# zhanxw/rvtests

Hardware: AMD Instinct MI355X
Metric: gene-sets/sec (SKAT+SKAT-O+CMC+Zeggini, analytic p-values) (higher is better)
Workload: dtype f64

## Files before the change

### rvtests_amd/csrc/k2_hardcall.hip

```cpp
#include "suffstat_hc.hip.h"

namespace rvt {

void k2_launch_hc(int MT, dim3 grid, hipStream_t st, const GeneDesc* d_desc, NullTile nt, long long N, long long ld,
                  int d) {
  switch (MT) {
    case 1: hipLaunchKernelGGL((gene_suffstat_hc<1, 2, 4, false>), grid, dim3(64), 0, st, d_desc, nt, N, ld, d); break;
    case 2: hipLaunchKernelGGL((gene_suffstat_hc<2, 2, 3, false>), grid, dim3(64), 0, st, d_desc, nt, N, ld, d); break;
    case 3: hipLaunchKernelGGL((gene_suffstat_hc<3, 2, 2, false>), grid, dim3(64), 0, st, d_desc, nt, N, ld, d); break;
    case 4: hipLaunchKernelGGL((gene_suffstat_hc<4, 2, 2, false>), grid, dim3(64), 0, st, d_desc, nt, N, ld, d); break;
    case 5: hipLaunchKernelGGL((gene_suffstat_hc<5, 1, 1, false>), grid, dim3(64), 0, st, d_desc, nt, N, ld, d); break;
    case 6: hipLaunchKernelGGL((gene_suffstat_hc<6, 1, 1, false>), grid, dim3(64), 0, st, d_desc, nt, N, ld, d); break;
    default: break;
  }
}

void k2_launch_classify(dim3 grid, hipStream_t st, const double* G, long long N, long long ld, int M, int* flag) {
  hipLaunchKernelGGL(block_classify_kernel<0>, grid, dim3(256), 0, st, G, N, ld, M, flag);
}

}
```

### rvtests_amd/csrc/suffstat_hc.hip.h

```cpp
#pragma once
#include <type_traits>
#include "suffstat_kernels.hip.h"

namespace rvt {

typedef int i4_t __attribute__((ext_vector_type(4)));
typedef unsigned int u4_t __attribute__((ext_vector_type(4)));

constexpr int kHcMaxMT = 6;
constexpr int kHcMaxD = 13;
constexpr int kHcStepUnit = 12;
constexpr int kHcMaxSteps = 1020;
constexpr int kHcColstatRows = 6;

constexpr int hc_pq_tiles(int MT) { return MT * MT + MT * (MT + 1) / 2; }
constexpr int hc_pq_words(int MT) { return hc_pq_tiles(MT) * 128; }
constexpr int hc_lds_words(int MT) { return hc_pq_words(MT) + 64 * MT + 4; }

struct NullTile {
  const double* base;
  int cols;
};

__device__ __forceinline__ unsigned row16_sum(unsigned h) {
  h += (unsigned)__builtin_amdgcn_update_dpp(0, (int)h, 0xB1, 0xF, 0xF, true);
  h += (unsigned)__builtin_amdgcn_update_dpp(0, (int)h, 0x4E, 0xF, 0xF, true);
  h += (unsigned)__builtin_amdgcn_update_dpp(0, (int)h, 0x141, 0xF, 0xF, true);
  h += (unsigned)__builtin_amdgcn_update_dpp(0, (int)h, 0x140, 0xF, 0xF, true);
  return h;
}

template <int MT>
struct HcStep {
  u4_t glo[MT], ghi[MT];
  u4_t xlo, xhi;
};

template <int MT, bool NT>
__device__ __forceinline__ void hc_issue(HcStep<MT>& f, const __amdgpu_buffer_rsrc_t& rg, const unsigned (&voff)[MT],
                                         const __amdgpu_buffer_rsrc_t& rx, unsigned xoff, int imm) {
#pragma unroll
  for (int c = 0; c < MT; ++c) {
    f.glo[c] = __builtin_bit_cast(u4_t, __builtin_amdgcn_raw_buffer_load_b128(rg, voff[c] + imm, 0, NT ? 2 : 0));
    f.ghi[c] = __builtin_bit_cast(u4_t, __builtin_amdgcn_raw_buffer_load_b128(rg, voff[c] + imm + 16, 0, NT ? 2 : 0));
  }
  f.xlo = __builtin_bit_cast(u4_t, __builtin_amdgcn_raw_buffer_load_b128(rx, xoff + imm, 0, 0));
  f.xhi = __builtin_bit_cast(u4_t, __builtin_amdgcn_raw_buffer_load_b128(rx, xoff + imm + 16, 0, 0));
}

__device__ __forceinline__ double hc_dbl(unsigned lo, unsigned hi) {
  return __builtin_bit_cast(double, ((unsigned long long)hi << 32) | lo);
}

struct HcBurden {
  double a_cmc, a_zeg;
  unsigned zz, cnt;
};

template <bool MASKED>
__device__ __forceinline__ void hc_row(const u4_t& glo, const u4_t& ghi, const double (&xv)[4], d4_t& accT,
                                       unsigned& pk, unsigned& mk, unsigned& cs, unsigned fx, unsigned& h, bool valid) {
  const double g0 = hc_dbl(glo[0], glo[1]), g1 = hc_dbl(glo[2], glo[3]), g2 = hc_dbl(ghi[0], ghi[1]),
               g3 = hc_dbl(ghi[2], ghi[3]);
  accT = __builtin_amdgcn_mfma_f64_16x16x4f64(g0, xv[0], accT, 0, 0, 0);
  accT = __builtin_amdgcn_mfma_f64_16x16x4f64(g1, xv[1], accT, 0, 0, 0);
  accT = __builtin_amdgcn_mfma_f64_16x16x4f64(g2, xv[2], accT, 0, 0, 0);
  accT = __builtin_amdgcn_mfma_f64_16x16x4f64(g3, xv[3], accT, 0, 0, 0);
  const unsigned w01 = __builtin_amdgcn_perm(glo[3], glo[1], 0x0c0c0703u);
  const unsigned w23 = __builtin_amdgcn_perm(ghi[3], ghi[1], 0x07030c0cu);
  unsigned p = ((w01 | w23) >> 5) & 0x03030303u;
  constexpr unsigned kAdd = 0x00100000u, kBits = 0xBFEFFFFFu;
  const unsigned i0 = ((glo[1] + kAdd) & kBits) | glo[0], i1 = ((glo[3] + kAdd) & kBits) | glo[2],
                 i2 = ((ghi[1] + kAdd) & kBits) | ghi[0], i3 = ((ghi[3] + kAdd) & kBits) | ghi[2];
  auto one = [](unsigned x) { return x < 1u ? x : 1u; };
  unsigned m = one(i0) | (one(i1) << 8) | (one(i2) << 16) | (one(i3) << 24);
  if (MASKED) {
    p = valid ? p : 0u;
    m = valid ? m : 0u;
  }
  const unsigned m3 = m * 3u;
  p &= ~m3;
  pk = p;
  mk = m;
  cs = __builtin_amdgcn_sad_u8(p, 0u, cs);
  const unsigned t = (p ^ fx) & ~m3;
  h += (t | (t >> 1)) & 0x01010101u;
}
__device__ __forceinline__ unsigned hc_code3(unsigned p) { return p & (p >> 1) & 0x01010101u; }

__device__ __forceinline__ void hc_note_masked(const u4_t& glo, const u4_t& ghi, unsigned mk, unsigned* oa) {
  auto note = [&](unsigned lo, unsigned hi) {
    __hip_atomic_fetch_or(oa + 0, lo, __ATOMIC_RELAXED, __HIP_MEMORY_SCOPE_WORKGROUP);
    __hip_atomic_fetch_or(oa + 1, hi, __ATOMIC_RELAXED, __HIP_MEMORY_SCOPE_WORKGROUP);
    __hip_atomic_fetch_and(oa + 2, lo, __ATOMIC_RELAXED, __HIP_MEMORY_SCOPE_WORKGROUP);
    __hip_atomic_fetch_and(oa + 3, hi, __ATOMIC_RELAXED, __HIP_MEMORY_SCOPE_WORKGROUP);
  };
  if (mk & 0x000000ffu) note(glo[0], glo[1]);
  if (mk & 0x0000ff00u) note(glo[2], glo[3]);
  if (mk & 0x00ff0000u) note(ghi[0], ghi[1]);
  if (mk & 0xff000000u) note(ghi[2], ghi[3]);
}

template <bool MASKED>
__device__ __forceinline__ void hc_finish(unsigned h, const double (&xv)[4], HcBurden& bu, unsigned vmask) {
  h = row16_sum(h);
  if (MASKED) h &= vmask;
#pragma unroll
  for (int l = 0; l < 4; ++l) {
    const unsigned cz = (h >> (8 * l)) & 0xffu;
    const unsigned cc = cz ? 1u : 0u;
    bu.zz = cz * cz + bu.zz;
    bu.cnt += cc;
    bu.a_zeg = fma((double)cz, xv[l], bu.a_zeg);
    bu.a_cmc = fma((double)cc, xv[l], bu.a_cmc);
  }
}

struct HcMaskCtx {
  unsigned* oa;
  unsigned* flag;
};

template <int MT, bool MASKED>
__device__ __forceinline__ void hc_step(const HcStep<MT>& f, const int T, d4_t (&accT)[MT], unsigned (&pk)[MT][4],
                                        unsigned (&cs)[MT], const unsigned (&fx)[MT], HcBurden& bu, bool valid,
                                        unsigned vmask, unsigned& anym, const HcMaskCtx& mc) {
  double xv[4] = {hc_dbl(f.xlo[0], f.xlo[1]), hc_dbl(f.xlo[2], f.xlo[3]), hc_dbl(f.xhi[0], f.xhi[1]),
                  hc_dbl(f.xhi[2], f.xhi[3])};
  if (MASKED) {
#pragma unroll
    for (int l = 0; l < 4; ++l) xv[l] = valid ? xv[l] : 0.0;
  }
  unsigned h = 0;
#pragma unroll
  for (int c = 0; c < MT; ++c) {
    unsigned p, m;
    hc_row<MASKED>(f.glo[c], f.ghi[c], xv, accT[c], p, m, cs[c], fx[c], h, valid);
    if (m) hc_note_masked(f.glo[c], f.ghi[c], m, mc.oa + 64 * c);
    if (hc_code3(p)) __hip_atomic_fetch_or(mc.flag, 2u, __ATOMIC_RELAXED, __HIP_MEMORY_SCOPE_WORKGROUP);
    pk[c][T] = p | (m << 2);
    anym |= m;
  }
  hc_finish<MASKED>(h, xv, bu, vmask);
}

template <int MT>
__device__ __forceinline__ void hc_gram(const unsigned (&pk)[MT][4], i4_t (&accS)[MT * (MT + 1) / 2]) {
  i4_t op[MT];
#pragma unroll
  for (int c = 0; c < MT; ++c) op[c] = i4_t{(int)pk[c][0], (int)pk[c][1], (int)pk[c][2], (int)pk[c][3]};
  int t = 0;
#pragma unroll
  for (int r = 0; r < MT; ++r)
#pragma unroll
    for (int c = r; c < MT; ++c, ++t) accS[t] = __builtin_amdgcn_mfma_i32_16x16x64_i8(op[r], op[c], accS[t], 0, 0, 0);
}

template <int MT>
__device__ __forceinline__ void hc_gram_masked(const unsigned (&pk)[MT][4], unsigned* lds, int lane) {
  auto mask_op = [&](int c) {
    return i4_t{(int)((pk[c][0] >> 2) & 0x01010101u), (int)((pk[c][1] >> 2) & 0x01010101u),
                (int)((pk[c][2] >> 2) & 0x01010101u), (int)((pk[c][3] >> 2) & 0x01010101u)};
  };
  auto add = [&](int tile, const i4_t& z) {
    const unsigned w0 = (unsigned)z[0] | ((unsigned)z[1] << 16), w1 = (unsigned)z[2] | ((unsigned)z[3] << 16);
    __hip_atomic_fetch_add(lds + (tile * 2 + 0) * 64 + lane, w0, __ATOMIC_RELAXED, __HIP_MEMORY_SCOPE_WORKGROUP);
    __hip_atomic_fetch_add(lds + (tile * 2 + 1) * 64 + lane, w1, __ATOMIC_RELAXED, __HIP_MEMORY_SCOPE_WORKGROUP);
  };
#pragma unroll
  for (int c = 0; c < MT; ++c) {
    const i4_t mc = mask_op(c);
#pragma unroll
    for (int r = 0; r < MT; ++r) {
      const i4_t a = i4_t{(int)pk[r][0], (int)pk[r][1], (int)pk[r][2], (int)pk[r][3]};
      add(r * MT + c, __builtin_amdgcn_mfma_i32_16x16x64_i8(a, mc, i4_t{0, 0, 0, 0}, 0, 0, 0));
      if (r <= c) {
        const i4_t mr = (r == c) ? mc : mask_op(r);
        add(MT * MT + r * MT - r * (r - 1) / 2 + (c - r), __builtin_amdgcn_mfma_i32_16x16x64_i8(mr, mc, i4_t{0, 0, 0, 0}, 0, 0, 0));
      }
    }
    __builtin_amdgcn_sched_barrier(0);
  }
  __hip_atomic_fetch_or(lds + hc_pq_words(MT) + 64 * MT, 1u, __ATOMIC_RELAXED, __HIP_MEMORY_SCOPE_WORKGROUP);
}

template <int MT>
__device__ __forceinline__ void hc_group_end(const unsigned (&pk)[MT][4], i4_t (&accS)[MT * (MT + 1) / 2], unsigned& anym,
                                             unsigned* lds, int lane) {
  hc_gram<MT>(pk, accS);
  if (__builtin_amdgcn_ballot_w64(anym != 0u) != 0ull) hc_gram_masked<MT>(pk, lds, lane);
  anym = 0u;
}

template <int MT, int DEPTH, bool NT>
__device__ __forceinline__ void suffstat_hc_body(const GeneDesc& gd, const NullTile& nt, long long N, long long ld,
                                                 int d, unsigned* lds) {
  const int lane = threadIdx.x & 63;
  const int v = lane & 15, q = lane >> 4;
  const int wpart = blockIdx.x;
  if (wpart >= gd.n_wparts) return;
  constexpr int kPQ = hc_pq_words(MT);
#pragma unroll 4
  for (int w = lane; w < kPQ; w += 64) lds[w] = 0u;
#pragma unroll
  for (int c = 0; c < MT; ++c) lds[kPQ + 64 * c + lane] = (lane & 2) ? 0xffffffffu : 0u;
  if (lane < 4) lds[kPQ + 64 * MT + lane] = 0u;
  const HcMaskCtx mc{lds + kPQ + 4 * v, lds + kPQ + 64 * MT};
  unsigned anym = 0u;
  const long long nsteps = ld >> 4;
  const long long s_begin = (long long)wpart * gd.steps_per_wpart;
  long long s_end = s_begin + gd.steps_per_wpart;
  if (s_end > nsteps) s_end = nsteps;
  if (s_begin >= s_end) return;
  const int M = gd.M;
  auto uniform = [](const void* p) {
    const unsigned long long a = (unsigned long long)p;
    const unsigned lo = __builtin_amdgcn_readfirstlane((unsigned)a);
    const unsigned hi = __builtin_amdgcn_readfirstlane((unsigned)(a >> 32));
    return (void*)(((unsigned long long)hi << 32) | lo);
  };
  const unsigned gbytes = (unsigned)((unsigned long long)M * (unsigned long long)ld * 8ull);
  const __amdgpu_buffer_rsrc_t rg = __builtin_amdgcn_make_buffer_rsrc(uniform(gd.G), 0, gbytes, 0x00020000);
  const unsigned xbytes = (unsigned)((unsigned long long)nt.cols * (unsigned long long)ld * 8ull);
  const __amdgpu_buffer_rsrc_t rx = __builtin_amdgcn_make_buffer_rsrc(uniform(nt.base), 0, xbytes, 0x00020000);
  const unsigned lane_off = (unsigned)(q * 32);
  const unsigned col_bytes = (unsigned)((unsigned long long)ld * 8ull);
  unsigned vbase[MT];
#pragma unroll
  for (int c = 0; c < MT; ++c) {
    const int col = c * 16 + v;
    vbase[c] = (col < M) ? (unsigned)col * col_bytes + lane_off : 0x80000000u;
  }
  const int xcol = (v <= d) ? v : d + 1;
  const unsigned xbase = (unsigned)xcol * col_bytes + lane_off;
  unsigned fx[MT];
#pragma unroll
  for (int c = 0; c < MT; ++c) fx[c] = ((gd.pflip[c] >> v) & 1) ? 0x02020202u : 0u;

  d4_t accT[MT];
  i4_t accS[MT * (MT + 1) / 2];
  unsigned cs[MT], pk[MT][4];
#pragma unroll
  for (int c = 0; c < MT; ++c) {
    accT[c] = d4_t{0.0, 0.0, 0.0, 0.0};
    cs[c] = 0;
  }
#pragma unroll
  for (int t = 0; t < MT * (MT + 1) / 2; ++t) accS[t] = i4_t{0, 0, 0, 0};
  HcBurden bu{0.0, 0.0, 0u, 0u};

  long long s = s_begin;
  const long long full = N >> 4;
  const long long s_fast_end = (s_end < full) ? s_end : full;
  constexpr int U = (DEPTH == 3) ? 12 : 4;
  const long long n_fast = (s_fast_end > s_begin) ? (s_fast_end - s_begin) / U : 0;
  if constexpr (DEPTH == 1) {
   if (n_fast > 0) {
    unsigned voff[MT];
#pragma unroll
    for (int c = 0; c < MT; ++c) voff[c] = vbase[c] + (unsigned)(s_begin * 128);
    unsigned xoff = xbase + (unsigned)(s_begin * 128);
    u4_t glo[MT], ghi[MT], xlo[2], xhi[2];
#pragma unroll
    for (int c = 0; c < MT; ++c) {
      glo[c] = __builtin_bit_cast(u4_t, __builtin_amdgcn_raw_buffer_load_b128(rg, voff[c], 0, NT ? 2 : 0));
      ghi[c] = __builtin_bit_cast(u4_t, __builtin_amdgcn_raw_buffer_load_b128(rg, voff[c] + 16, 0, NT ? 2 : 0));
    }
    xlo[0] = __builtin_bit_cast(u4_t, __builtin_amdgcn_raw_buffer_load_b128(rx, xoff, 0, 0));
    xhi[0] = __builtin_bit_cast(u4_t, __builtin_amdgcn_raw_buffer_load_b128(rx, xoff + 16, 0, 0));
    for (long long it = 0; it < n_fast; ++it) {
#pragma unroll
      for (int u = 0; u < 4; ++u) {
        xlo[(u + 1) & 1] = __builtin_bit_cast(u4_t, __builtin_amdgcn_raw_buffer_load_b128(rx, xoff + (u + 1) * 128, 0, 0));
        xhi[(u + 1) & 1] = __builtin_bit_cast(u4_t, __builtin_amdgcn_raw_buffer_load_b128(rx, xoff + (u + 1) * 128 + 16, 0, 0));
        __builtin_amdgcn_sched_barrier(0);
        const double xv[4] = {hc_dbl(xlo[u & 1][0], xlo[u & 1][1]), hc_dbl(xlo[u & 1][2], xlo[u & 1][3]),
                              hc_dbl(xhi[u & 1][0], xhi[u & 1][1]), hc_dbl(xhi[u & 1][2], xhi[u & 1][3])};
        unsigned h = 0;
#pragma unroll
        for (int c = 0; c < MT; ++c) {
          unsigned p, m;
          hc_row<false>(glo[c], ghi[c], xv, accT[c], p, m, cs[c], fx[c], h, true);
          if (m) hc_note_masked(glo[c], ghi[c], m, mc.oa + 64 * c);
          if (hc_code3(p)) __hip_atomic_fetch_or(mc.flag, 2u, __ATOMIC_RELAXED, __HIP_MEMORY_SCOPE_WORKGROUP);
          pk[c][u] = p | (m << 2);
          anym |= m;
          glo[c] = __builtin_bit_cast(u4_t, __builtin_amdgcn_raw_buffer_load_b128(rg, voff[c] + (u + 1) * 128, 0, NT ? 2 : 0));
          ghi[c] = __builtin_bit_cast(u4_t, __builtin_amdgcn_raw_buffer_load_b128(rg, voff[c] + (u + 1) * 128 + 16, 0, NT ? 2 : 0));
          __builtin_amdgcn_sched_barrier(0);
        }
        hc_finish<false>(h, xv, bu, 0xffffffffu);
        if (u == 3) hc_group_end<MT>(pk, accS, anym, lds, lane);
        __builtin_amdgcn_sched_barrier(0);
      }
#pragma unroll
      for (int c = 0; c < MT; ++c) voff[c] += 4 * 128;
      xoff += 4 * 128;
    }
    s += n_fast * U;
   }
  } else if (n_fast > 0) {
    unsigned voff[MT];
#pragma unroll
    for (int c = 0; c < MT; ++c) voff[c] = vbase[c] + (unsigned)(s_begin * 128);
    unsigned xoff = xbase + (unsigned)(s_begin * 128);
    HcStep<MT> f[DEPTH];
#pragma unroll
    for (int u = 0; u < DEPTH - 1; ++u) hc_issue<MT, NT>(f[u], rg, voff, rx, xoff, u * 128);
    for (long long it = 0; it < n_fast; ++it) {
#pragma unroll
      for (int u = 0; u < U; ++u) {
        hc_issue<MT, NT>(f[(u + DEPTH - 1) % DEPTH], rg, voff, rx, xoff, (u + DEPTH - 1) * 128);
        __builtin_amdgcn_sched_barrier(0);
        hc_step<MT, false>(f[u % DEPTH], u & 3, accT, pk, cs, fx, bu, true, 0xffffffffu, anym, mc);
        if ((u & 3) == 3) hc_group_end<MT>(pk, accS, anym, lds, lane);
        __builtin_amdgcn_sched_barrier(0);
      }
#pragma unroll
      for (int c = 0; c < MT; ++c) voff[c] += U * 128;
      xoff += U * 128;
    }
    s += n_fast * U;
  }
  while (s < s_end) {
#pragma unroll
    for (int c = 0; c < MT; ++c) pk[c][0] = pk[c][1] = pk[c][2] = pk[c][3] = 0u;
    auto one = [&](const int T, long long su) {
      const bool valid = su < s_end;
      const long long sc = valid ? su : s_end - 1;
      unsigned voff[MT];
#pragma unroll
      for (int c = 0; c < MT; ++c) voff[c] = vbase[c] + (unsigned)(sc * 128);
      HcStep<MT> f;
      hc_issue<MT, false>(f, rg, voff, rx, xbase + (unsigned)(sc * 128), 0);
      unsigned vmask = 0u;
      const long long smp = sc * 16 + q * 4;
#pragma unroll
      for (int l = 0; l < 4; ++l) vmask |= (valid && smp + l < N) ? (0xffu << (8 * l)) : 0u;
      hc_step<MT, true>(f, T, accT, pk, cs, fx, bu, valid, vmask, anym, mc);
    };
    one(0, s);
    one(1, s + 1);
    one(2, s + 2);
    one(3, s + 3);
    hc_group_end<MT>(pk, accS, anym, lds, lane);
    s += 4;
  }

  double* out = gd.parts + (long long)wpart * gd.Mp * gd.Cp;
  const int Cp = gd.Cp;
  {
    int t = 0;
#pragma unroll
    for (int r = 0; r < MT; ++r)
#pragma unroll
      for (int c = r; c < MT; ++c, ++t) {
        const int col = c * 16 + v;
        if (col < M) {
#pragma unroll
          for (int i = 0; i < 4; ++i) out[(long long)(r * 16 + q * 4 + i) * Cp + col] = (double)accS[t][i];
        }
      }
  }
#pragma unroll
  for (int r = 0; r < MT; ++r) {
#pragma unroll
    for (int i = 0; i < 4; ++i) {
      const int row = r * 16 + q + 4 * i;
      if (M + v < Cp) out[(long long)row * Cp + M + v] = accT[r][i];
      if (M + 16 + v < Cp) out[(long long)row * Cp + M + 16 + v] = 0.0;
    }
  }
  long long cnt_w = ((s_end * 16 < N) ? s_end * 16 : N) - s_begin * 16;
  if (cnt_w < 0) cnt_w = 0;
  double* cst = gd.colstat + (long long)wpart * kHcColstatRows * gd.Mp;
  const unsigned wflag = lds[kPQ + 64 * MT];
  {
    int t = 0;
#pragma unroll
    for (int c = 0; c < MT; ++c) {
      unsigned sc = cs[c];
      sc += __shfl_xor(sc, 16, 64);
      sc += __shfl_xor(sc, 32, 64);
      const i4_t dg = accS[t];
      const int sel = (lane & 3) == 0 ? dg[0] : ((lane & 3) == 1 ? dg[1] : ((lane & 3) == 2 ? dg[2] : dg[3]));
      const int diag = __shfl(sel, v + 16 * (v >> 2), 64);
      const int tq = MT * MT + t;
      const unsigned qw = lds[(tq * 2 + ((v >> 1) & 1)) * 64 + v + 16 * (v >> 2)];
      const long long nm = (long long)((qw >> (16 * (v & 1))) & 0xffffu);
      t += MT - c;
      const long long sm = (long long)sc, hh = (long long)diag - 16 * nm, n2 = (hh - sm) / 2, n1 = 2 * sm - hh,
                      n0 = cnt_w - n1 - n2 - nm;
      const double mn = n0 > 0 ? 0.0 : (n1 > 0 ? 1.0 : (n2 > 0 ? 2.0 : INFINITY));
      const double mx = n2 > 0 ? 2.0 : (n1 > 0 ? 1.0 : (n0 > 0 ? 0.0 : -INFINITY));
      if (lane < 16) {
        const int j = c * 16 + lane;
        cst[j] = (double)sm;
        cst[gd.Mp + j] = mn;
        cst[2 * gd.Mp + j] = mx;
        cst[3 * gd.Mp + j] = (double)nm;
        const unsigned* w = lds + kPQ + 64 * c + 4 * lane;
        unsigned long long* bits = reinterpret_cast<unsigned long long*>(cst);
        bits[4 * gd.Mp + j] = ((unsigned long long)w[1] << 32) | w[0];
        bits[5 * gd.Mp + j] = ((unsigned long long)w[3] << 32) | w[2];
      }
    }
  }
  if (gd.wflags && lane == 0) gd.wflags[wpart] = wflag;
  if ((wflag & 1u) && gd.pq) {
    unsigned* dst = gd.pq + (long long)wpart * kPQ;
#pragma unroll 4
    for (int w = lane; w < kPQ; w += 64) dst[w] = lds[w];
  }
  if (gd.bparts) {
    double ac = bu.a_cmc, az = bu.a_zeg;
    ac += __shfl_xor(ac, 16, 64);
    az += __shfl_xor(az, 16, 64);
    ac += __shfl_xor(ac, 32, 64);
    az += __shfl_xor(az, 32, 64);
    unsigned zz = bu.zz, cn = bu.cnt;
    zz += __shfl_xor(zz, 16, 64);
    cn += __shfl_xor(cn, 16, 64);
    zz += __shfl_xor(zz, 32, 64);
    cn += __shfl_xor(cn, 32, 64);
    const int rl = 3 + d;
    double* bp = gd.bparts + (long long)wpart * 2 * rl;
    if (lane <= d) {
      const int k = (lane == d) ? 0 : 3 + lane;
      bp[k] = ac;
      bp[rl + k] = az;
    }
    if (lane == 0) {
      bp[1] = (double)cn;
      bp[2] = (double)cn;
      bp[rl + 1] = (double)zz;
      bp[rl + 2] = (double)cn;
    }
  }
}

template <int MT, int DEPTH, int WAVES, bool NT>
__global__ __launch_bounds__(64, WAVES) void gene_suffstat_hc(const GeneDesc* __restrict__ genes, NullTile nt,
                                                              long long N, long long ld, int d) {
  __shared__ unsigned lds[hc_lds_words(MT)];
  const GeneDesc gd = genes[blockIdx.y];
  if (gd.MT != MT) return;
  suffstat_hc_body<MT, DEPTH, NT>(gd, nt, N, ld, d, lds);
}

template <int UNUSED = 0>
__global__ __launch_bounds__(256) void block_classify_kernel(const double* __restrict__ G, long long N, long long ld,
                                                             int M, int* __restrict__ flag) {
  const long long per_col = (N + 1) / 2;
  const long long total = per_col * M;
  bool bad = false;
  for (long long idx = blockIdx.x * (long long)blockDim.x + threadIdx.x; idx < total;
       idx += (long long)gridDim.x * blockDim.x) {
    const long long j = idx / per_col, i = (idx % per_col) * 2;
    const unsigned long long* p = reinterpret_cast<const unsigned long long*>(G + j * ld + i);
    const unsigned long long a = p[0], b = (i + 1 < N) ? p[1] : 0ull;
    auto ok = [](unsigned long long x) {
      return x == 0ull || x == 0x3FF0000000000000ull || x == 0x4000000000000000ull;
    };
    bad |= !ok(a) || !ok(b);
  }
  if (__any(bad) && (threadIdx.x & 63) == 0) atomicAnd(flag, 0);
}

}
```

Before: 25820.

## Share null-tile loads across genes via LDS ring in multi-wave hardcall kernel

Adds a shared variant of the hardcall sufficient-statistics kernel. It packs W=4 genes into one workgroup, and all waves cooperatively stage the null-model covariate tile into a double-buffered LDS ring. Each wave then reads X from LDS instead of issuing its own global loads. The goal is to cut redundant global traffic for the shared X matrix. In exchange it adds block-wide barriers and extra LDS use, and waves whose gene does not match MT must still run the barriers. By default it is enabled only for MT=1, and an env var can override that.

New measurement: 25940, median of 6. No clear change (+0.5%).

```diff
diff --git a/rvtests_amd/csrc/k2_hardcall.hip b/rvtests_amd/csrc/k2_hardcall.hip
--- a/rvtests_amd/csrc/k2_hardcall.hip
+++ b/rvtests_amd/csrc/k2_hardcall.hip
@@ -1,9 +1,10 @@
+#include <cstdlib>
 #include "suffstat_hc.hip.h"
 
 namespace rvt {
 
-void k2_launch_hc(int MT, dim3 grid, hipStream_t st, const GeneDesc* d_desc, NullTile nt, long long N, long long ld,
-                  int d) {
+static void launch_hc_one(int MT, dim3 grid, hipStream_t st, const GeneDesc* d_desc, NullTile nt, long long N, long long ld,
+                          int d) {
   switch (MT) {
     case 1: hipLaunchKernelGGL((gene_suffstat_hc<1, 2, 4, false>), grid, dim3(64), 0, st, d_desc, nt, N, ld, d); break;
     case 2: hipLaunchKernelGGL((gene_suffstat_hc<2, 2, 3, false>), grid, dim3(64), 0, st, d_desc, nt, N, ld, d); break;
@@ -15,6 +16,36 @@
   }
 }
 
+constexpr int kHcSharedW = 4;
+static void launch_hc_shared(int MT, dim3 grid, hipStream_t st, const GeneDesc* d_desc, NullTile nt, long long N,
+                             long long ld, int d, int sl) {
+  const int n_run = (int)grid.y;
+  const dim3 g(grid.x, (n_run + kHcSharedW - 1) / kHcSharedW), b(64 * kHcSharedW);
+  switch (MT) {
+    case 1: hipLaunchKernelGGL((gene_suffstat_hc_shared<1, 2, 4, kHcSharedW>), g, b, 0, st, d_desc, n_run, nt, N, ld, d, sl); break;
+    case 2: hipLaunchKernelGGL((gene_suffstat_hc_shared<2, 2, 3, kHcSharedW>), g, b, 0, st, d_desc, n_run, nt, N, ld, d, sl); break;
+    case 3: hipLaunchKernelGGL((gene_suffstat_hc_shared<3, 2, 2, kHcSharedW>), g, b, 0, st, d_desc, n_run, nt, N, ld, d, sl); break;
+    case 4: hipLaunchKernelGGL((gene_suffstat_hc_shared<4, 2, 2, kHcSharedW>), g, b, 0, st, d_desc, n_run, nt, N, ld, d, sl); break;
+    case 5: hipLaunchKernelGGL((gene_suffstat_hc_shared<5, 1, 1, kHcSharedW>), g, b, 0, st, d_desc, n_run, nt, N, ld, d, sl); break;
+    case 6: hipLaunchKernelGGL((gene_suffstat_hc_shared<6, 1, 1, kHcSharedW>), g, b, 0, st, d_desc, n_run, nt, N, ld, d, sl); break;
+    default: break;
+  }
+}
+
+static const bool kHcSharedClass[kHcMaxMT + 1] = {false, true, false, false, false, false, false};
+
+void k2_launch_hc(int MT, dim3 grid, hipStream_t st, const GeneDesc* d_desc, NullTile nt, long long N, long long ld,
+                  int d) {
+  if (MT < 1 || MT > kHcMaxMT) return;
+  bool shared = kHcSharedClass[MT];
+  if (const char* e = getenv("RVT_HC_SHARED")) shared = atoi(e) != 0;
+  const int sl = hc_stage_log2(kHcSharedW, d);
+  if (shared && sl >= 0 && grid.y > 0)
+    launch_hc_shared(MT, grid, st, d_desc, nt, N, ld, d, sl);
+  else
+    launch_hc_one(MT, grid, st, d_desc, nt, N, ld, d);
+}
+
 void k2_launch_classify(dim3 grid, hipStream_t st, const double* G, long long N, long long ld, int M, int* flag) {
   hipLaunchKernelGGL(block_classify_kernel<0>, grid, dim3(256), 0, st, G, N, ld, M, flag);
 }
diff --git a/rvtests_amd/csrc/suffstat_hc.hip.h b/rvtests_amd/csrc/suffstat_hc.hip.h
--- a/rvtests_amd/csrc/suffstat_hc.hip.h
+++ b/rvtests_amd/csrc/suffstat_hc.hip.h
@@ -122,6 +122,24 @@
 };
 
 template <int MT, bool MASKED>
+__device__ __forceinline__ void hc_step_x(const u4_t (&glo)[MT], const u4_t (&ghi)[MT], const double (&xv)[4], const int T,
+                                          d4_t (&accT)[MT], unsigned (&pk)[MT][4], unsigned (&cs)[MT],
+                                          const unsigned (&fx)[MT], HcBurden& bu, bool valid, unsigned vmask,
+                                          unsigned& anym, const HcMaskCtx& mc) {
+  unsigned h = 0;
+#pragma unroll
+  for (int c = 0; c < MT; ++c) {
+    unsigned p, m;
+    hc_row<MASKED>(glo[c], ghi[c], xv, accT[c], p, m, cs[c], fx[c], h, valid);
+    if (m) hc_note_masked(glo[c], ghi[c], m, mc.oa + 64 * c);
+    if (hc_code3(p)) __hip_atomic_fetch_or(mc.flag, 2u, __ATOMIC_RELAXED, __HIP_MEMORY_SCOPE_WORKGROUP);
+    pk[c][T] = p | (m << 2);
+    anym |= m;
+  }
+  hc_finish<MASKED>(h, xv, bu, vmask);
+}
+
+template <int MT, bool MASKED>
 __device__ __forceinline__ void hc_step(const HcStep<MT>& f, const int T, d4_t (&accT)[MT], unsigned (&pk)[MT][4],
                                         unsigned (&cs)[MT], const unsigned (&fx)[MT], HcBurden& bu, bool valid,
                                         unsigned vmask, unsigned& anym, const HcMaskCtx& mc) {
@@ -131,17 +149,7 @@
 #pragma unroll
     for (int l = 0; l < 4; ++l) xv[l] = valid ? xv[l] : 0.0;
   }
-  unsigned h = 0;
-#pragma unroll
-  for (int c = 0; c < MT; ++c) {
-    unsigned p, m;
-    hc_row<MASKED>(f.glo[c], f.ghi[c], xv, accT[c], p, m, cs[c], fx[c], h, valid);
-    if (m) hc_note_masked(f.glo[c], f.ghi[c], m, mc.oa + 64 * c);
-    if (hc_code3(p)) __hip_atomic_fetch_or(mc.flag, 2u, __ATOMIC_RELAXED, __HIP_MEMORY_SCOPE_WORKGROUP);
-    pk[c][T] = p | (m << 2);
-    anym |= m;
-  }
-  hc_finish<MASKED>(h, xv, bu, vmask);
+  hc_step_x<MT, MASKED>(f.glo, f.ghi, xv, T, accT, pk, cs, fx, bu, valid, vmask, anym, mc);
 }
 
 template <int MT>
@@ -192,9 +200,57 @@
   anym = 0u;
 }
 
-template <int MT, int DEPTH, bool NT>
+constexpr int kHcNullChunks = 2;
+constexpr int hc_ring_bytes(int W) { return kHcNullChunks * W * 64 * 16 + (kHcMaxD + 1) * 64; }
+inline int hc_stage_log2(int W, int d) {
+  for (int sl = 4; sl >= 2; --sl)
+    if ((8 << sl) <= W * 64 && (d + 1) * (8 << sl) <= kHcNullChunks * W * 64) return sl;
+  return -1;
+}
+
+template <int W>
+struct HcNullLoader {
+  unsigned goff;
+  unsigned loff;
+  unsigned gstep, lstep;
+  unsigned npieces;
+  u4_t r[kHcNullChunks];
+  unsigned stage_bytes;
+  __device__ __forceinline__ void init(int d, int sl, unsigned col_bytes, long long s_begin) {
+    const unsigned cstride = (128u << sl) + 64u;
+    stage_bytes = 128u << sl;
+    const unsigned col = threadIdx.x >> (sl + 3), off = threadIdx.x & ((8u << sl) - 1u);
+    const unsigned dcol = (unsigned)(W * 64) >> (sl + 3);
+    goff = col * col_bytes + off * 16u + (unsigned)(s_begin * 128);
+    loff = col * cstride + off * 16u;
+    gstep = dcol * col_bytes;
+    lstep = dcol * cstride;
+    npieces = col <= (unsigned)d ? ((unsigned)d - col) / dcol + 1u : 0u;
+  }
+  __device__ __forceinline__ void fetch(const __amdgpu_buffer_rsrc_t& rx) {
+#pragma unroll
+    for (int j = 0; j < kHcNullChunks; ++j)
+      r[j] = __builtin_bit_cast(u4_t, __builtin_amdgcn_raw_buffer_load_b128(rx, (unsigned)j < npieces ? goff + j * gstep : 0x80000000u, 0, 0));
+    goff += stage_bytes;
+  }
+  __device__ __forceinline__ void put(unsigned char* buf) const {
+#pragma unroll
+    for (int j = 0; j < kHcNullChunks; ++j)
+      if ((unsigned)j < npieces) *reinterpret_cast<u4_t*>(buf + loff + j * lstep) = r[j];
+  }
+};
+
+__device__ __forceinline__ void hc_xv(double (&xv)[4], const u4_t& lo, const u4_t& hi, bool xon) {
+  xv[0] = xon ? hc_dbl(lo[0], lo[1]) : 0.0;
+  xv[1] = xon ? hc_dbl(lo[2], lo[3]) : 0.0;
+  xv[2] = xon ? hc_dbl(hi[0], hi[1]) : 0.0;
+  xv[3] = xon ? hc_dbl(hi[2], hi[3]) : 0.0;
+}
+
+template <int MT, int DEPTH, bool NT, int W = 1>
 __device__ __forceinline__ void suffstat_hc_body(const GeneDesc& gd, const NullTile& nt, long long N, long long ld,
-                                                 int d, unsigned* lds) {
+                                                 int d, unsigned* lds, unsigned char* ring = nullptr, int sl = 0,
+                                                 bool active = true) {
   const int lane = threadIdx.x & 63;
   const int v = lane & 15, q = lane >> 4;
   const int wpart = blockIdx.x;
@@ -231,8 +287,7 @@
     const int col = c * 16 + v;
     vbase[c] = (col < M) ? (unsigned)col * col_bytes + lane_off : 0x80000000u;
   }
-  const int xcol = (v <= d) ? v : d + 1;
-  const unsigned xbase = (unsigned)xcol * col_bytes + lane_off;
+  const unsigned xbase = (v <= d) ? (unsigned)v * col_bytes + lane_off : 0x80000000u;
   unsigned fx[MT];
 #pragma unroll
   for (int c = 0; c < MT; ++c) fx[c] = ((gd.pflip[c] >> v) & 1) ? 0x02020202u : 0u;
@@ -254,7 +309,118 @@
   const long long s_fast_end = (s_end < full) ? s_end : full;
   constexpr int U = (DEPTH == 3) ? 12 : 4;
   const long long n_fast = (s_fast_end > s_begin) ? (s_fast_end - s_begin) / U : 0;
-  if constexpr (DEPTH == 1) {
+  if constexpr (W > 1) {
+   static_assert(DEPTH <= 2, "the shared form works in groups of 4 steps");
+   if (n_fast > 0) {
+    constexpr int kBuf = hc_ring_bytes(W);
+    HcNullLoader<W> nl;
+    nl.init(d, sl, col_bytes, s_begin);
+    const long long F = n_fast * U;
+    const int nstages = (int)((F + (1 << sl) - 1) >> sl);
+    nl.fetch(rx);
+    nl.put(ring);
+    __syncthreads();
+    if (!active) {
+      for (int k = 0; k < nstages; ++k) {
+        const bool more = k + 1 < nstages;
+        if (more) {
+          nl.fetch(rx);
+          nl.put(ring + ((k + 1) & 1) * kBuf);
+        }
+        __syncthreads();
+      }
+      return;
+    }
+    const bool xon = v <= d;
+    const unsigned xrd = (unsigned)(xon ? v : 0) * ((128u << sl) + 64u) + lane_off;
+    unsigned voff[MT];
+#pragma unroll
+    for (int c = 0; c < MT; ++c) voff[c] = vbase[c] + (unsigned)(s_begin * 128);
+    auto ldx = [](const unsigned char* p) { return *reinterpret_cast<const u4_t*>(p); };
+    if constexpr (DEPTH == 1) {
+      u4_t glo[MT], ghi[MT];
+#pragma unroll
+      for (int c = 0; c < MT; ++c) {
+        glo[c] = __builtin_bit_cast(u4_t, __builtin_amdgcn_raw_buffer_load_b128(rg, voff[c], 0, NT ? 2 : 0));
+        ghi[c] = __builtin_bit_cast(u4_t, __builtin_amdgcn_raw_buffer_load_b128(rg, voff[c] + 16, 0, NT ? 2 : 0));
+      }
+      for (int k = 0; k < nstages; ++k) {
+        const bool more = k + 1 < nstages;
+        if (more) nl.fetch(rx);
+        const long long left = F - ((long long)k << sl);
+        const int nit = (int)((left < (1 << sl) ? left : (1 << sl)) >> 2);
+        const unsigned char* rb = ring + (k & 1) * kBuf + xrd;
+        for (int it = 0; it < nit; ++it) {
+#pragma unroll
+          for (int u = 0; u < 4; ++u) {
+            const u4_t xlo = ldx(rb + u * 128), xhi = ldx(rb + u * 128 + 16);
+            if (u == 3 && more && it == nit - 1) nl.put(ring + ((k + 1) & 1) * kBuf);
+            __builtin_amdgcn_sched_barrier(0);
+            double xv[4];
+            hc_xv(xv, xlo, xhi, xon);
+            unsigned h = 0;
+#pragma unroll
+            for (int c = 0; c < MT; ++c) {
+              unsigned p, m;
+              hc_row<false>(glo[c], ghi[c], xv, accT[c], p, m, cs[c], fx[c], h, true);
+              if (m) hc_note_masked(glo[c], ghi[c], m, mc.oa + 64 * c);
+              if (hc_code3(p)) __hip_atomic_fetch_or(mc.flag, 2u, __ATOMIC_RELAXED, __HIP_MEMORY_SCOPE_WORKGROUP);
+              pk[c][u] = p | (m << 2);
+              anym |= m;
+              glo[c] = __builtin_bit_cast(u4_t, __builtin_amdgcn_raw_buffer_load_b128(rg, voff[c] + (u + 1) * 128, 0, NT ? 2 : 0));
+              ghi[c] = __builtin_bit_cast(u4_t, __builtin_amdgcn_raw_buffer_load_b128(rg, voff[c] + (u + 1) * 128 + 16, 0, NT ? 2 : 0));
+              __builtin_amdgcn_sched_barrier(0);
+            }
+            hc_finish<false>(h, xv, bu, 0xffffffffu);
+            if (u == 3) hc_group_end<MT>(pk, accS, anym, lds, lane);
+            __builtin_amdgcn_sched_barrier(0);
+          }
+#pragma unroll
+          for (int c = 0; c < MT; ++c) voff[c] += 4 * 128;
+          rb += 4 * 128;
+        }
+        __syncthreads();
+      }
+    } else {
+      u4_t glo[2][MT], ghi[2][MT];
+      auto issue_g = [&](int b, int imm) {
+#pragma unroll
+        for (int c = 0; c < MT; ++c) {
+          glo[b][c] = __builtin_bit_cast(u4_t, __builtin_amdgcn_raw_buffer_load_b128(rg, voff[c] + imm, 0, NT ? 2 : 0));
+          ghi[b][c] = __builtin_bit_cast(u4_t, __builtin_amdgcn_raw_buffer_load_b128(rg, voff[c] + imm + 16, 0, NT ? 2 : 0));
+        }
+      };
+      issue_g(0, 0);
+      for (int k = 0; k < nstages; ++k) {
+        const bool more = k + 1 < nstages;
+        if (more) nl.fetch(rx);
+        const long long left = F - ((long long)k << sl);
+        const int nit = (int)((left < (1 << sl) ? left : (1 << sl)) >> 2);
+        const unsigned char* rb = ring + (k & 1) * kBuf + xrd;
+        for (int it = 0; it < nit; ++it) {
+#pragma unroll
+          for (int u = 0; u < 4; ++u) {
+            issue_g((u + 1) & 1, (u + 1) * 128);
+            const u4_t xlo = ldx(rb + u * 128), xhi = ldx(rb + u * 128 + 16);
+            if (u == 3 && more && it == nit - 1) nl.put(ring + ((k + 1) & 1) * kBuf);
+            __builtin_amdgcn_sched_barrier(0);
+            double xv[4];
+            hc_xv(xv, xlo, xhi, xon);
+            hc_step_x<MT, false>(glo[u & 1], ghi[u & 1], xv, u, accT, pk, cs, fx, bu, true, 0xffffffffu, anym, mc);
+            if (u == 3) hc_group_end<MT>(pk, accS, anym, lds, lane);
+            __builtin_amdgcn_sched_barrier(0);
+          }
+#pragma unroll
+          for (int c = 0; c < MT; ++c) voff[c] += 4 * 128;
+          rb += 4 * 128;
+        }
+        __syncthreads();
+      }
+    }
+    s += F;
+   }
+   if (!active) return;
+  } else if constexpr (DEPTH == 1) {
    if (n_fast > 0) {
     unsigned voff[MT];
 #pragma unroll
@@ -448,6 +614,18 @@
   suffstat_hc_body<MT, DEPTH, NT>(gd, nt, N, ld, d, lds);
 }
 
+template <int MT, int DEPTH, int WAVES, int W>
+__global__ __launch_bounds__(64 * W, WAVES) void gene_suffstat_hc_shared(const GeneDesc* __restrict__ genes, int n_run,
+                                                                         NullTile nt, long long N, long long ld, int d,
+                                                                         int sl) {
+  __shared__ unsigned lds[W][hc_lds_words(MT)];
+  __shared__ __attribute__((aligned(16))) unsigned char ring[2 * hc_ring_bytes(W)];
+  const int w = __builtin_amdgcn_readfirstlane((int)(threadIdx.x >> 6));
+  const int g = (int)blockIdx.y * W + w;
+  const GeneDesc gd = genes[g < n_run ? g : n_run - 1];
+  suffstat_hc_body<MT, DEPTH, false, W>(gd, nt, N, ld, d, lds[w], ring, sl, g < n_run && gd.MT == MT);
+}
+
 template <int UNUSED = 0>
 __global__ __launch_bounds__(256) void block_classify_kernel(const double* __restrict__ G, long long N, long long ld,
                                                              int M, int* __restrict__ flag) {
```
